# qkniep/alpenglow

Measured on AMD Instinct MI355X. Metric: GiB/s device-resident RS shred encode+reconstruct, batched 1 MiB blocks, higher is better.
Workload: dtype u8 (GF(2^16) symbols, bitsliced u32 planes); 1 GPU; 4096 x 1 MiB blocks per GPU, 32:32 encode + reconstruct with 16/32 data shreds erased; blocks_per_gpu=4096, block_bytes=1048576, data_shreds=32, coding_shreds=32, erased_data_shreds=16, lost_coding_shreds=0, random_patterns=False, parallelism=blocks sharded over 1 GPU(s), no collective, only=both

## Files before the change

### alpenglow_amd/csrc/rs_decode_pk.hpp

```cpp
#pragma once
#include <hip/hip_runtime.h>

#include "rs_device.hpp"
#include "rs_launch.hpp"
#include "rs_xform.hpp"

namespace ag {
namespace {

using dev::static_for;

__device__ __forceinline__ uint32_t m65535_add(uint32_t a, uint32_t b) {
  const uint32_t s = a + b;
  return s >= 65535u ? s - 65535u : s;
}
__device__ __forceinline__ uint32_t m65535_sub(uint32_t a, uint32_t b) { return a >= b ? a - b : a + 65535u - b; }
__device__ __forceinline__ uint32_t m65535_mul(uint32_t a, uint32_t b) {
  const uint32_t p = a * b;
  uint32_t s = (p & 0xFFFFu) + (p >> 16);
  s = (s & 0xFFFFu) + (s >> 16);
  return s >= 65535u ? s - 65535u : s;
}
__device__ __forceinline__ uint32_t walsh64(uint32_t v, int lane) {
  static_for<6>([&](auto B) {
    constexpr int d = 1 << decltype(B)::value;
    const uint32_t o = static_cast<uint32_t>(__shfl_xor(static_cast<int>(v), d));
    v = (lane & d) ? m65535_sub(o, v) : m65535_add(v, o);
  });
  return v;
}
__device__ __forceinline__ void walsh128(uint32_t& v0, uint32_t& v1, int lane) {
  v0 = walsh64(v0, lane);
  v1 = walsh64(v1, lane);
  const uint32_t a = v0;
  v0 = m65535_add(a, v1);
  v1 = m65535_sub(a, v1);
}
__device__ __forceinline__ uint16_t locator_log(uint32_t loc, bool in) {
  return static_cast<uint16_t>(in ? loc : 65535u - loc);
}

struct PkShared {
  uint32_t lcoef[2 * 64];
  uint64_t smask[2][2];
  uint8_t ilist[2][64], olist[2][64];
};
struct PkLocTables {
  uint16_t log64[64];
  uint16_t apow_lo[256], apow_hi[256];
};
__device__ __forceinline__ uint32_t poly_mul(uint32_t a, uint32_t b) {
  uint32_t r = 0;
  for (int i = 0; i < 16; ++i) r ^= ((b >> i) & 1) ? a << i : 0u;
  for (int i = 30; i >= 16; --i) r ^= ((r >> i) & 1) ? (1u << i) ^ (0x2Du << (i - 16)) : 0u;
  return r;
}
__device__ __forceinline__ uint32_t poly_pow_a(const PkLocTables& t, uint32_t l) {
  return poly_mul(t.apow_hi[l >> 8], t.apow_lo[l & 255]);
}

template <int OUTH, bool SRV = false, bool TAIL = false>
__device__ __forceinline__ void decode_pk_tile(const DecodeXParams& p, uint32_t tile, uint4* lds, X8Flags* fl,
                                               PkShared& sh, const PkLocTables* loc = nullptr) {
  static_assert(OUTH >= -1 && OUTH <= 1, "OUTH: the restored positions' window half, -1 both");
  constexpr int W = 64, kSl = 16;
  constexpr int D = 2;
  X8Flags& flags = *fl;
  uint32_t* lcoef = sh.lcoef;
  auto& smask = sh.smask;
  auto& ilist = sh.ilist;
  auto& olist = sh.olist;
  const int lane = threadIdx.x & 63;
  const int h = lane >> 5;
  const int wave = __builtin_amdgcn_readfirstlane(threadIdx.x >> 6);
  const uint64_t sb0 = static_cast<uint64_t>(tile) * 2;
  const uint64_t nblk = p.total_columns / kSl;
  const uint32_t opos = p.low_rate ? 0 : p.chunk, rpos = p.low_rate ? p.chunk : 0;
  if (threadIdx.x < 2 * W) {
    const uint32_t sl = threadIdx.x >> 6, j = threadIdx.x & 63;
    uint64_t im = 0, om = 0;
    if (sb0 + sl < nblk) {
      im = p.pmask[2 * (sb0 + sl)];
      om = p.pmask[2 * (sb0 + sl) + 1];
      if constexpr (SRV) {
        const uint64_t e = ~im;
        const uint32_t hl = m65535_mul(walsh64(j ? loc->log64[j] : 0u, static_cast<int>(j)), 1024u);
        const uint32_t hi = walsh64(static_cast<uint32_t>((e >> j) & 1), static_cast<int>(j));
        const uint32_t acc = walsh64(m65535_mul(hl, hi), static_cast<int>(j));
        lcoef[threadIdx.x] = poly_pow_a(*loc, locator_log(acc, (im >> j) & 1));
      } else if (((im | om) >> j) & 1) {
        lcoef[threadIdx.x] = p.rows[(sb0 + sl) * p.rows_w + j];
      }
    }
    const uint64_t below = (uint64_t{1} << j) - 1;
    if ((im >> j) & 1) ilist[sl][__builtin_popcountll(im & below)] = static_cast<uint8_t>(j);
    if ((om >> j) & 1) olist[sl][__builtin_popcountll(om & below)] = static_cast<uint8_t>(j);
    if (j == 0) {
      smask[sl][0] = im;
      smask[sl][1] = om;
    }
  }
  if (threadIdx.x < 16) reinterpret_cast<uint32_t*>(&flags)[threadIdx.x] = 0;
  __syncthreads();
  const uint64_t imA = smask[0][0], imB = smask[1][0], omA = smask[0][1], omB = smask[1][1];
  const uint32_t nA = static_cast<uint32_t>(__builtin_popcountll(imA));
  const uint32_t nin = nA + static_cast<uint32_t>(__builtin_popcountll(imB));
  const uint32_t noA = static_cast<uint32_t>(__builtin_popcountll(omA));
  const uint32_t nout = noA + static_cast<uint32_t>(__builtin_popcountll(omB));
  if (nout == 0) return;
  const int col = lane & 15, row = lane >> 4;
  const bool tail_lane = TAIL && col == kSl - 1;
  auto src_of = [&](uint32_t sl, uint32_t g) -> const uint8_t* {
    const bool is_rec = p.low_rate ? g >= p.chunk : g < p.chunk;
    const uint64_t blk = sb0 + sl;
    return is_rec ? p.rec + (g - rpos) * p.rec_shard_stride + blk * p.rec_block_stride + col * 64
                  : p.orig + (g - opos) * p.orig_shard_stride + blk * p.orig_block_stride + col * 64;
  };
  uint32_t v[2][16];
  static_for<2>([&](auto U) {
    constexpr int u = decltype(U)::value;
    const uint32_t i = u * 32 + wave * 4 + row;
    if (i < nin) {
      const uint32_t sl = i < nA ? 0u : 1u;
      const uint8_t* src = src_of(sl, ilist[sl][i - (sl ? nA : 0u)]);
      if (tail_lane) {
        load_tail_chunk(src, p.tail_bytes, v[u]);
      } else {
        static_for<4>([&](auto Q) {
          constexpr int q = decltype(Q)::value;
          const uint4 x = ld_piece(src + 16 * q);
          v[u][4 * q] = x.x;
          v[u][4 * q + 1] = x.y;
          v[u][4 * q + 2] = x.z;
          v[u][4 * q + 3] = x.w;
        });
      }
    } else {
      static_for<16>([&](auto P) { v[u][decltype(P)::value] = 0; });
    }
  });
  static_for<2>([&](auto U) {
    constexpr int u = decltype(U)::value;
    if (static_cast<uint32_t>(u * 32 + wave * 4) < nin) {
      const uint32_t i = u * 32 + wave * 4 + row;
      const bool ok = i < nin;
      const uint32_t sl = i < nA ? 0u : 1u;
      const uint32_t j = ok ? ilist[sl][i - (sl ? nA : 0u)] : 0u;
      dev::planes_from_raw(v[u]);
      dev::mul_rt_poly(v[u], lcoef[sl * W + j]);
      if (ok) {
        static_for<4>([&](auto Q) {
          constexpr int q = decltype(Q)::value;
          lds[(i * 4 + q) * kSl + col] = make_uint4(v[u][4 * q], v[u][4 * q + 1], v[u][4 * q + 2], v[u][4 * q + 3]);
        });
      }
    }
  });
  __syncthreads();
  const uint32_t lsl = static_cast<uint32_t>((lane & 31) >> 4);
  const uint64_t in_mask = lsl ? imB : imA, out_mask = lsl ? omB : omA;
  auto posA = [&](int t) -> uint32_t {
    return static_cast<uint32_t>((t & 1) | ((t >> 1) << 1) | (h << 2) | (wave << 3));
  };
  Regs4 r;
  static_for<4>([&](auto T) {
    constexpr int t = decltype(T)::value;
    const uint32_t j = posA(t);
    if ((in_mask >> j) & 1) {
      const uint32_t i = static_cast<uint32_t>(__builtin_popcountll(in_mask & ((uint64_t{1} << j) - 1))) + (lsl ? nA : 0u);
      static_for<4>([&](auto Q) {
        constexpr int q = decltype(Q)::value;
        const uint4 x = lds[(i * 4 + q) * kSl + col];
        r[t][4 * q] = x.x;
        r[t][4 * q + 1] = x.y;
        r[t][4 * q + 2] = x.z;
        r[t][4 * q + 3] = x.w;
      });
    } else {
      static_for<16>([&](auto P) { r[t][decltype(P)::value] = 0; });
    }
  });
  __syncthreads();
  h8_layer0<true, 0, 1>(wave, h, r);
  h8_relayout(r);
  x8_layer_t<LB, 1, true, 0, 1>(wave, r);
  x8_layer_t<LB, 2, true, 0, 1>(wave, r);
  x8_swap<1, 0, 1, 0xF, false>(wave, lane, lds, &flags, r);
  x8_layer_t<LC, 3, true, 0, 1>(wave, r);
  x8_swap<0, 1, 2, 0xF, false>(wave, lane, lds, &flags, r);
  x8_layer_t<LD, 4, true, 0, 1>(wave, r);
  x8_swap<1, 2, 3, 0xF, false>(wave, lane, lds, &flags, r);
  x8_layer_t<LE, 5, true, 0, 1>(wave, r);
  auto wait_readers = [&](int x, uint32_t e) __attribute__((always_inline)) {
    static_for<3>([&](auto Bb) {
      constexpr int b = decltype(Bb)::value;
      if ((x >> b) & 1) x8_wait_ge(&flags.done[x & ~(1 << b)], e);
    });
  };
  static_for<2>([&](auto Rho) {
    constexpr int rho = decltype(Rho)::value;
    constexpr uint32_t e = 4 + rho;
    if constexpr (rho == 1) wait_readers(wave, e - 1);
    static_for<2>([&](auto U) { lds_put(lds, 2 * wave + decltype(U)::value, lane, r[2 * rho + decltype(U)::value]); });
    x8_signal(&flags.ready[wave], e, lane);
    static_for<2>([&](auto U) {
      constexpr int t = 2 * rho + decltype(U)::value;
      uint32_t hi[16];
      static_for<16>([&](auto P) {
        constexpr int q = decltype(P)::value;
        hi[q] = __builtin_amdgcn_permlane32_swap(r[t][q], 0u, false, false)[1];
      });
      if constexpr (!(t & 1)) dev::xor_planes(r[t], r[t | 1]);
      if constexpr (!(t & 2)) dev::xor_planes(r[t], r[t | 2]);
      dev::xor_planes(r[t], hi);
    });
    static_for<3>([&](auto Bb) {
      constexpr int b = decltype(Bb)::value;
      if (!((wave >> b) & 1)) {
        const int pw = wave | (1 << b);
        x8_wait_ge(&flags.ready[pw], e);
        static_for<2>([&](auto U) { lds_get_xor(lds, 2 * pw + decltype(U)::value, lane, r[2 * rho + decltype(U)::value]); });
      }
    });
    x8_signal(&flags.done[wave], e, lane);
  });
  x8_layer_t<LE, 5, false, 0, 1>(wave, r);
  x8_layer_t<LE, 4, false, 0, 1>(wave, r);
  wait_readers(wave ^ 4, 5);
  if constexpr (OUTH < 0) {
    x8_swap<1, 2, 4 + D, 0xF, false>(wave, lane, lds, &flags, r);
  } else {
    const int partner = wave ^ 4;
    if (((wave >> 2) & 1) != OUTH) {
      x8_wait_ge(&flags.done[partner], 3 + D);
      static_for<4>([&](auto T) {
        constexpr int t = decltype(T)::value;
        if constexpr (((t >> 1) & 1) == OUTH) {
          lds_put(lds, 2 * partner + (t & 1), lane, r[t]);
          __asm__ volatile("; pk put %0" ::"n"(t));
        }
      });
      x8_signal(&flags.ready[wave], 4 + D, lane);
      return;
    }
    x8_wait_ge(&flags.ready[partner], 4 + D);
    static_for<4>([&](auto T) {
      constexpr int t = decltype(T)::value;
      if constexpr (((t >> 1) & 1) != OUTH) {
        lds_get(lds, 2 * wave + (t & 1), lane, r[t]);
        __asm__ volatile("; pk get %0" ::"n"(t));
      }
    });
    x8_signal(&flags.done[wave], 4 + D, lane);
  }
  x8_layer_t<LD, 3, false, 0, 1>(wave, r);
  x8_swap<0, 1, 5 + D, 0xF, false>(wave, lane, lds, &flags, r);
  x8_layer_t<LC, 2, false, 0, 1>(wave, r);
  x8_swap<1, 0, 6 + D, 0xF, false>(wave, lane, lds, &flags, r);
  x8_layer_t<LB, 1, false, 0, 1>(wave, r);
  h8_relayout(r);
  h8_layer0<false, 0, 1>(wave, h, r);
  constexpr int kLive = OUTH < 0 ? 8 : 4;
  constexpr int kHi = OUTH < 0 ? 0 : OUTH << 2;
  const int lw = wave & (kLive - 1);
  static_for<kLive>([&](auto Wv) {
    constexpr int w2 = decltype(Wv)::value;
    x8_wait_ge(&flags.done[w2 | kHi], 6 + D);
  });
  static_for<4>([&](auto T) {
    constexpr int t = decltype(T)::value;
    uint32_t j = posA(t);
    __asm__ volatile("" : "+v"(j));
    if ((out_mask >> j) & 1) {
      const uint32_t o = static_cast<uint32_t>(__builtin_popcountll(out_mask & ((uint64_t{1} << j) - 1))) + (lsl ? noA : 0u);
      static_for<4>([&](auto Q) {
        constexpr int q = decltype(Q)::value;
        lds[(o * 4 + q) * kSl + col] = make_uint4(r[t][4 * q], r[t][4 * q + 1], r[t][4 * q + 2], r[t][4 * q + 3]);
      });
    }
  });
  x8_signal(&flags.ready[wave], 7 + D, lane);
  static_for<kLive>([&](auto Wv) {
    constexpr int w2 = decltype(Wv)::value;
    x8_wait_ge(&flags.ready[w2 | kHi], 7 + D);
  });
  constexpr int kPer = 64 / kLive;
  static_for<kPer / 4>([&](auto U) {
    constexpr int u = decltype(U)::value;
    if (static_cast<uint32_t>(u * 4 * kLive + lw * 4) < nout) {
      const uint32_t o = u * 4 * kLive + lw * 4 + row;
      if (o < nout) {
        const uint32_t sl = o < noA ? 0u : 1u;
        const uint32_t j = olist[sl][o - (sl ? noA : 0u)];
        uint32_t v[16];
        static_for<4>([&](auto Q) {
          constexpr int q = decltype(Q)::value;
          const uint4 x = lds[(o * 4 + q) * kSl + col];
          v[4 * q] = x.x;
          v[4 * q + 1] = x.y;
          v[4 * q + 2] = x.z;
          v[4 * q + 3] = x.w;
        });
        dev::mul_rt_poly(v, lcoef[sl * W + j]);
        if (tail_lane) {
          dev::transpose8(v);
          dev::transpose8(v + 8);
          store_tail_chunk(const_cast<uint8_t*>(src_of(sl, j)), p.tail_bytes, v);
        } else {
          dev::store_chunk<true>(const_cast<uint8_t*>(src_of(sl, j)), v);
        }
      }
    }
  });
}

}

}
```

Measured before the change: 1582 GiB/s.

## Coalesce decode tile loads and stores into full lines with in-register exchange

Changes global loads and stores in the decode tile so each 16-byte piece of a lane group lands in a contiguous 256-byte line (address src - col*48 + 256*q) rather than each lane reading its own 64 contiguous bytes. The data is then reshuffled with a quad_exchange across lanes, or through an LDS round-trip fallback, before the bitslice transform. This is meant to improve memory coalescing for the bandwidth-bound encode/reconstruct path. The cost is extra cross-lane shuffles, and it relies on quad_exchange existing and being correct for the layout.

```diff
diff --git a/alpenglow_amd/csrc/rs_decode_pk.hpp b/alpenglow_amd/csrc/rs_decode_pk.hpp
--- a/alpenglow_amd/csrc/rs_decode_pk.hpp
+++ b/alpenglow_amd/csrc/rs_decode_pk.hpp
@@ -59,10 +59,38 @@
   return poly_mul(t.apow_hi[l >> 8], t.apow_lo[l & 255]);
 }
 
+constexpr int kPkIoStoreLines = 1;
+constexpr int kPkIoLoadLines = 2;
+constexpr int kPkIoPlainStores = 4;
+template <bool TO_PIECES>
+__device__ __forceinline__ void pk_via_item(uint4* item, int col, uint32_t* x) {
+  static_for<4>([&](auto Q) {
+    constexpr int q = decltype(Q)::value;
+    item[TO_PIECES ? col * 4 + q : 16 * q + col] = make_uint4(x[4 * q], x[4 * q + 1], x[4 * q + 2], x[4 * q + 3]);
+  });
+  __builtin_amdgcn_fence(__ATOMIC_ACQ_REL, "wavefront");
+  __builtin_amdgcn_wave_barrier();
+  static_for<4>([&](auto Q) {
+    constexpr int q = decltype(Q)::value;
+    const uint4 y = item[TO_PIECES ? 16 * q + col : col * 4 + q];
+    x[4 * q] = y.x;
+    x[4 * q + 1] = y.y;
+    x[4 * q + 2] = y.z;
+    x[4 * q + 3] = y.w;
+  });
+  __builtin_amdgcn_fence(__ATOMIC_ACQ_REL, "wavefront");
+  __builtin_amdgcn_wave_barrier();
+}
+#ifndef AG_PK_IO
+#define AG_PK_IO (kPkIoStoreLines | kPkIoLoadLines)
+#endif
 template <int OUTH, bool SRV = false, bool TAIL = false>
 __device__ __forceinline__ void decode_pk_tile(const DecodeXParams& p, uint32_t tile, uint4* lds, X8Flags* fl,
                                                PkShared& sh, const PkLocTables* loc = nullptr) {
   static_assert(OUTH >= -1 && OUTH <= 1, "OUTH: the restored positions' window half, -1 both");
+  constexpr int IO = (SRV || TAIL) ? 0 : AG_PK_IO;
+  constexpr bool kLdLines = (IO & kPkIoLoadLines) != 0, kStLines = (IO & kPkIoStoreLines) != 0;
+  constexpr bool kStNT = (IO & kPkIoPlainStores) == 0;
   constexpr int W = 64, kSl = 16;
   constexpr int D = 2;
   X8Flags& flags = *fl;
@@ -128,11 +156,19 @@
       } else {
         static_for<4>([&](auto Q) {
           constexpr int q = decltype(Q)::value;
-          const uint4 x = ld_piece(src + 16 * q);
-          v[u][4 * q] = x.x;
-          v[u][4 * q + 1] = x.y;
-          v[u][4 * q + 2] = x.z;
-          v[u][4 * q + 3] = x.w;
+          if constexpr (kLdLines) {
+            const uint4 x = ld_piece(src - col * 48 + 256 * q);
+            v[u][4 * q] = x.x;
+            v[u][4 * q + 1] = x.y;
+            v[u][4 * q + 2] = x.z;
+            v[u][4 * q + 3] = x.w;
+          } else {
+            const uint4 x = ld_piece(src + 16 * q);
+            v[u][4 * q] = x.x;
+            v[u][4 * q + 1] = x.y;
+            v[u][4 * q + 2] = x.z;
+            v[u][4 * q + 3] = x.w;
+          }
         });
       }
     } else {
@@ -146,6 +182,10 @@
       const bool ok = i < nin;
       const uint32_t sl = i < nA ? 0u : 1u;
       const uint32_t j = ok ? ilist[sl][i - (sl ? nA : 0u)] : 0u;
+      if constexpr (kLdLines && kStLines) quad_exchange(v[u], lane);
+      else if constexpr (kLdLines) {
+        if (ok) pk_via_item<false>(lds + i * 64, col, v[u]);
+      }
       dev::planes_from_raw(v[u]);
       dev::mul_rt_poly(v[u], lcoef[sl * W + j]);
       if (ok) {
@@ -306,8 +346,22 @@
           dev::transpose8(v);
           dev::transpose8(v + 8);
           store_tail_chunk(const_cast<uint8_t*>(src_of(sl, j)), p.tail_bytes, v);
+        } else if constexpr (kStLines) {
+          dev::transpose8(v);
+          dev::transpose8(v + 8);
+          if constexpr (kLdLines) quad_exchange(v, lane);
+          else pk_via_item<true>(lds + o * 64, col, v);
+          uint8_t* dst = const_cast<uint8_t*>(src_of(sl, j)) - col * 48;
+          static_for<4>([&](auto Q) {
+            constexpr int q = decltype(Q)::value;
+            if constexpr (kStNT) {
+              st_piece(dst + 256 * q, v[4 * q], v[4 * q + 1], v[4 * q + 2], v[4 * q + 3]);
+            } else {
+              *reinterpret_cast<dev::u32x4*>(dst + 256 * q) = dev::u32x4{v[4 * q], v[4 * q + 1], v[4 * q + 2], v[4 * q + 3]};
+            }
+          });
         } else {
-          dev::store_chunk<true>(const_cast<uint8_t*>(src_of(sl, j)), v);
+          dev::store_chunk<kStNT>(const_cast<uint8_t*>(src_of(sl, j)), v);
         }
       }
     }
```

After: 1580 GiB/s. Within noise of the previous version (-0.1%).
